# stefanch/sGDML

Measured on AMD Instinct MI355X. Metric: kernel-matrix build+solve wall-clock, N_train=1000 21-atom (aspirin-sized), lower is better.
Workload: dtype f64

## Files before the change

sgdml_amd/csrc/chol.hip:

```cpp
#include "common.h"
#include "tile_sched.h"
#include <array>
#include <type_traits>
#include <utility>

typedef double d4 __attribute__((ext_vector_type(4)));
typedef double d2 __attribute__((ext_vector_type(2)));

#define GT 128
#define GBK 16
#define GPITCH 17

struct GemmArgs {
  const double* A;
  const double* B;
  double* C;
  int64_t M, N, K, lda, ldb, ldc;
  int lower;
  int tiles_m, tiles_n;
  int64_t n_super;
  int64_t s_begin;
  int super_n;
  int aligned;
  int cyc_W, cyc_rank;
  int64_t cyc_lb0, cyc_nb, cyc_col0, cyc_block_rows;
  double* diagA;
  int diag_nbw;
  int64_t diag_off;
  int* diag_info;
  int col0_first;
  int* ready;
  int ready_target, ready_rows;
  const double* A2;
  const double* B2;
  double* C2;
  int64_t M2, N2, K2;
  int tiles2;
  int second_compact;
  int bal;
  TileLaunch tl;
};

__global__ void __launch_bounds__(256, 2) gemm_nt_sub_diag_kernel(GemmArgs g);

template <bool FULL>
__device__ __forceinline__ void gemm_load_tile(const double* __restrict__ G, int64_t ld,
                                               int64_t row0, int64_t nrows, int64_t k0, int64_t K,
                                               int tid, d2 (&r)[4]) {
#pragma unroll
  for (int s = 0; s < 4; ++s) {
    int cidx = tid + 256 * s;
    int row = cidx >> 3, kc = (cidx & 7) * 2;
    int64_t gr = row0 + row, gk = k0 + kc;
    if (FULL) {
      r[s] = *reinterpret_cast<const d2*>(G + gr * ld + gk);
// ... 205 lines not shown
  int64_t ti, tj;
  if (g.bal) {
    if (!tile_decode_bal(g.tl, b, &ti, &tj)) return;
  } else if (!tile_decode_super(b, g.lower, g.col0_first, g.tiles_m, g.tiles_n, g.super_n, g.s_begin, g.n_super, &ti, &tj)) {
    return;
  }
  const int64_t row0 = ti * GT, col0 = tj * GT;
  if (g.cyc_W > 0 && row0 + GT <= g.cyc_block_rows) {
    const int64_t gb = (g.cyc_lb0 + row0 / g.cyc_nb) * g.cyc_W + g.cyc_rank;
    const int64_t grow_last = gb * g.cyc_nb + (row0 + GT - 1) % g.cyc_nb;
    if (g.cyc_col0 + col0 > grow_last) return;
  }
  const bool full = (row0 + GT <= g.M) && (col0 + GT <= g.N) && ((g.K & (GBK - 1)) == 0) && g.aligned;
  if (full)
    gemm_tile_body<true, OW>(g, lds, row0, col0);
  else
    gemm_tile_body<false, OW>(g, lds, row0, col0);
  if (g.ready && g.tiles2 == 0 && ti < g.ready_rows && tj < g.ready_rows) {
    __threadfence();
    __syncthreads();
    if (threadIdx.x == 0) atomicAdd(g.ready, 1);
  }
}

__global__ void __launch_bounds__(256, 2) gemm_nt_sub_kernel(GemmArgs g) {
  __shared__ __attribute__((aligned(16))) double lds[2][2][GT * GPITCH];
  gemm_block<false>(g, lds, blockIdx.x);
}


__global__ void __launch_bounds__(256, 2) gemm_nt_neg_kernel(GemmArgs g) {
  __shared__ __attribute__((aligned(16))) double lds[2][2][GT * GPITCH];
  gemm_block<true>(g, lds, blockIdx.x);
}

struct DiagJob {
  double* A = nullptr;
  int nbw = 0;
  int64_t off = 0;
  int* ready = nullptr;
  int ready_target = 0;
  bool col0_first = false;
  const double* A2 = nullptr;
  const double* B2 = nullptr;
  double* C2 = nullptr;
  int64_t M2 = 0, N2 = 0, K2 = 0;
  int64_t next_M2 = 0, next_N2 = 0, next_K2 = 0;
};

struct TileSchedEntry {
  TileSched S;
  const uint32_t* dev[2] = {nullptr, nullptr};
};
struct TileSchedCache {
  std::map<std::array<int64_t, 7>, TileSchedEntry> entries;
  char* block = nullptr;
  size_t cap = 0, used = 0;
};

void tile_sched_cache_free(gdml_ctx* ctx) {
  if (!ctx->tile_sched) return;
  if (ctx->tile_sched->block) hipFree(ctx->tile_sched->block);
  delete ctx->tile_sched;
  ctx->tile_sched = nullptr;
}

static int second_blocks(int64_t M2, int64_t N2, bool* compact) {
  const int64_t tm2 = ceil_div(M2, GT), tn2 = ceil_div(N2, GT);
  *compact = tm2 >= tn2;
  return (int)(tm2 * tn2 - (*compact ? tn2 * (tn2 - 1) / 2 : 0));
}

static int tile_sched_get(gdml_ctx* ctx, hipStream_t st, int tiles_m, int tiles_n, bool col0_first, int n_launch, int lead2,
                          int64_t K2, int64_t K, const TileSchedEntry** out) {
  *out = nullptr;
  if (!ctx->tile_sched) ctx->tile_sched = new TileSchedCache();
  TileSchedCache* c = ctx->tile_sched;
  const std::array<int64_t, 7> key = {tiles_m, tiles_n, col0_first ? 1 : 0, n_launch, lead2, lead2 ? K2 : 0, lead2 ? K : 0};
  auto it = c->entries.find(key);
  if (it == c->entries.end()) {
    TileSchedEntry e;
    double base[8] = {0, 0, 0, 0, 0, 0, 0, 0};
    for (int q = 0; q < lead2; ++q) base[((q - lead2) % 8 + 8) % 8] += (double)K2 / (double)K;
    tile_sched_build(tiles_m, tiles_n, col0_first, n_launch, base, &e.S);
    if (e.S.ok) {
      const size_t b0 = (e.S.table[0].size() * 4 + 255) & ~(size_t)255, b1 = (e.S.table[1].size() * 4 + 255) & ~(size_t)255;
      const size_t block_bytes = (size_t)8 << 20;
      if (!c->block) {
        HIP_CHECK(ctx, hipMalloc((void**)&c->block, block_bytes));
        c->cap = block_bytes;
      }
      if (b0 + b1 > c->cap) {
        e.S.ok = false;
      } else {
        if (c->used + b0 + b1 > c->cap) {
          HIP_CHECK(ctx, hipDeviceSynchronize());
          c->entries.clear();
          c->used = 0;
        }
        char* d = c->block + c->used;
        c->used += b0 + b1;
        if (!e.S.table[0].empty()) HIP_CHECK(ctx, hipMemcpyAsync(d, e.S.table[0].data(), e.S.table[0].size() * 4, hipMemcpyHostToDevice, st));
        if (!e.S.table[1].empty()) HIP_CHECK(ctx, hipMemcpyAsync(d + b0, e.S.table[1].data(), e.S.table[1].size() * 4, hipMemcpyHostToDevice, st));
        HIP_CHECK(ctx, hipStreamSynchronize(st));
        e.dev[0] = reinterpret_cast<const uint32_t*>(d);
        e.dev[1] = reinterpret_cast<const uint32_t*>(d + b0);
      }
    }
// ... 305 lines not shown
      d4 a[2][4], bb[2][4];
#pragma unroll
      for (int i = 0; i < 2; ++i)
#pragma unroll
        for (int ch = 0; ch < 4; ++ch) {
          a[i][ch] = *reinterpret_cast<const d4*>(Ap + (int64_t)(16 * i) * ld + 16 * ch);
          bb[i][ch] = *reinterpret_cast<const d4*>(Bp + (int64_t)(16 * i) * ld + 16 * ch);
        }
#pragma unroll
      for (int ch = 0; ch < 4; ++ch)
#pragma unroll
        for (int sidx = 0; sidx < 4; ++sidx)
#pragma unroll
          for (int i = 0; i < 2; ++i)
#pragma unroll
            for (int j = 0; j < 2; ++j)
              acc[i][j] = __builtin_amdgcn_mfma_f64_16x16x4f64(-a[i][ch][sidx], bb[j][ch][sidx], acc[i][j], 0, 0, 0);
#pragma unroll
      for (int i = 0; i < 2; ++i)
#pragma unroll
        for (int j = 0; j < 2; ++j)
#pragma unroll
          for (int r = 0; r < 4; ++r) Cp[(int64_t)(16 * i + 4 * r) * ld + 16 * j] = acc[i][j][r];
    }
    __syncthreads();
  }
}


__global__ void __launch_bounds__(256, 2) gemm_nt_sub_diag_kernel(GemmArgs g) {
  __shared__ __attribute__((aligned(16))) double lds[2][2][GT * GPITCH];
  static_assert(sizeof(double) * 2 * 2 * GT * GPITCH >= sizeof(double) * (2 * 64 * 65 + 64 + 128), "LDS of the diagonal role");
  if (blockIdx.x == 0) {
    if (g.ready) {
      if (threadIdx.x == 0) {
        int spins = 0;
        while (__hip_atomic_load(g.ready, __ATOMIC_RELAXED, __HIP_MEMORY_SCOPE_AGENT) < g.ready_target) {
          __builtin_amdgcn_s_sleep(8);
          if (++spins > (1 << 24)) {
            atomicExch(g.ready + 1, 1);
            break;
          }
        }
      }
      __syncthreads();
      __threadfence();
    }
    diag_block_role(g.diagA, g.ldc, g.diag_nbw, g.diag_off, g.diag_info, &lds[0][0][0]);
    return;
  }
  gemm_block<false>(g, lds, (int64_t)blockIdx.x - 1);
}

__global__ void __launch_bounds__(64) potrf64_kernel(double* __restrict__ A, int64_t ld, int w,
                                                     int64_t global_off, int* __restrict__ info) {
  __shared__ __attribute__((aligned(16))) double T[64 * 65];
  __shared__ __attribute__((aligned(16))) double col[64 * 8];
  const int lane = threadIdx.x;
  {
    double tv[64];
    const int lc = lane < w ? lane : w - 1;
#pragma unroll
    for (int r = 0; r < 64; ++r) tv[r] = A[(int64_t)(r < w ? r : w - 1) * ld + lc];
#pragma unroll
    for (int r = 0; r < 64; ++r) T[r * 65 + lane] = (r < w && lane < w) ? tv[r] : ((r == lane) ? 1.0 : 0.0);
  }
  __builtin_amdgcn_s_waitcnt(0xc07f);
  const int fail = potrf64_wave(T, col, lane);
  if (fail != 0 && fail <= w && lane == 0) atomicCAS(info, 0, (int)(global_off + fail));
  for (int r = 0; r < w; ++r)
    if (lane <= r && lane < w) A[(int64_t)r * ld + lane] = T[r * 65 + lane];
}

__global__ void __launch_bounds__(256) potrf_trsm64_kernel(double* __restrict__ A, double* __restrict__ X,
                                                           int64_t ld, int w, int64_t m, int64_t global_off,
                                                           int* __restrict__ info, double* __restrict__ Lsave,
                                                           const double* __restrict__ Lprev,
                                                           double* __restrict__ Aprev, int wprev) {
  __shared__ __attribute__((aligned(16))) double T[64 * 65];
  __shared__ __attribute__((aligned(16))) double Ls[64 * 64];
  __shared__ __attribute__((aligned(16))) double col[64 * 8];
  __shared__ double rinv[64];
  const int tid = threadIdx.x, lane = tid & 63, wave = tid >> 6;
  double pv[16];
  const bool wb = blockIdx.x == 0 && Lprev != nullptr;
  if (wb) {
#pragma unroll
    for (int i = 0; i < 16; ++i) pv[i] = Lprev[tid + 256 * i];
  }
  {
    double tv[16];
    const int lc = lane < w ? lane : w - 1;
#pragma unroll
    for (int i = 0; i < 16; ++i) {
      const int r = wave + 4 * i;
      tv[i] = A[(int64_t)(r < w ? r : w - 1) * ld + lc];
    }
#pragma unroll
    for (int i = 0; i < 16; ++i) {
      const int r = wave + 4 * i;
      T[r * 65 + lane] = (r < w && lane < w) ? tv[i] : ((r == lane) ? 1.0 : 0.0);
    }
  }
  if (wb) {
#pragma unroll
    for (int i = 0; i < 16; ++i) {
// ... 310 lines not shown
                                                            int skip_upper) {
  const int lane = threadIdx.x & 63, wave = threadIdx.x >> 6;
  const int li = lane & 15, lk = lane >> 4;
  const int tn = (ncols + 31) >> 5;
  const int t = blockIdx.x * 4 + wave;
  const int ti = t / tn, tj = t - ti * tn;
  if (32 * ti >= m) return;
  if (skip_upper && tj > ti) return;
  const int r0 = 32 * ti, q0 = 32 * tj;
  d4 acc[2][2], a[2][4], bb[2][4];
  int crow[2][4], ccol[2];
#pragma unroll
  for (int j = 0; j < 2; ++j) ccol[j] = q0 + 16 * j + li;
#pragma unroll
  for (int i = 0; i < 2; ++i)
#pragma unroll
    for (int r = 0; r < 4; ++r) crow[i][r] = r0 + 16 * i + lk + 4 * r;
#pragma unroll
  for (int i = 0; i < 2; ++i) {
    const int ra = r0 + 16 * i + li, rb = q0 + 16 * i + li;
    const double* Ap = A + (int64_t)(ra < m ? ra : m - 1) * ld + 4 * lk;
    const double* Bp = B + (int64_t)(rb < ncols ? rb : ncols - 1) * ld + 4 * lk;
#pragma unroll
    for (int ch = 0; ch < 4; ++ch) {
      a[i][ch] = *reinterpret_cast<const d4*>(Ap + 16 * ch);
      bb[i][ch] = *reinterpret_cast<const d4*>(Bp + 16 * ch);
    }
  }
#pragma unroll
  for (int i = 0; i < 2; ++i)
#pragma unroll
    for (int j = 0; j < 2; ++j)
#pragma unroll
      for (int r = 0; r < 4; ++r) {
        const int rr = crow[i][r] < m ? crow[i][r] : m - 1, cc = ccol[j] < ncols ? ccol[j] : ncols - 1;
        acc[i][j][r] = C[(int64_t)rr * ld + cc];
      }
#pragma unroll
  for (int ch = 0; ch < 4; ++ch)
#pragma unroll
    for (int sidx = 0; sidx < 4; ++sidx)
#pragma unroll
      for (int i = 0; i < 2; ++i)
#pragma unroll
        for (int j = 0; j < 2; ++j)
          acc[i][j] = __builtin_amdgcn_mfma_f64_16x16x4f64(-a[i][ch][sidx], bb[j][ch][sidx], acc[i][j], 0, 0, 0);
#pragma unroll
  for (int i = 0; i < 2; ++i)
#pragma unroll
    for (int j = 0; j < 2; ++j)
#pragma unroll
      for (int r = 0; r < 4; ++r)
        if (crow[i][r] < m && ccol[j] < ncols) C[(int64_t)crow[i][r] * ld + ccol[j]] = acc[i][j][r];
}

int panel_factor_steps(gdml_ctx* ctx, hipStream_t st, double* A, int64_t n, int64_t ld, int64_t k0, int64_t nb);

static int panel_factor(gdml_ctx* ctx, hipStream_t st, double* A, int64_t n, int64_t ld, int64_t k0,
                        int64_t nb) {
  const int64_t below = n - k0 - nb;
  const bool aligned = (reinterpret_cast<uintptr_t>(A) & 31) == 0 && (ld % 4 == 0) && (k0 % 4 == 0);
  if (nb % 64 == 0 && nb <= 512 && below > 0 && aligned) {
    GDML_TRY(panel_factor_steps(ctx, st, A, k0 + nb, ld, k0, nb));
    return launch_panel_trsm(ctx, st, A + k0 * ld + k0, A + (k0 + nb) * ld + k0, ld, (int)nb, below);
  }
  return panel_factor_steps(ctx, st, A, n, ld, k0, nb);
}

int panel_factor_steps(gdml_ctx* ctx, hipStream_t st, double* A, int64_t n, int64_t ld, int64_t k0,
                       int64_t nb) {
  double* save = nullptr;
  GDML_TRY(ctx_slot(ctx, SLOT_PANEL_SAVE, 2 * 4096 * 8, &save));
  const double* Lprev = nullptr;
  double* Aprev = nullptr;
  int wprev = 0, flip = 0;
  for (int64_t jj = 0; jj < nb; jj += 64) {
    const int64_t c0 = k0 + jj;
    const int w = (int)((nb - jj < 64) ? nb - jj : 64);
    double* Ad = A + c0 * ld + c0;
    const int64_t m = n - c0 - w;
    if (m > 0) {
      double* X = A + (c0 + w) * ld + c0;
      double* Lsave = save + flip * 4096;
      hipLaunchKernelGGL(potrf_trsm64_kernel, dim3((unsigned)ceil_div(m, 256)), dim3(256), 0, st, Ad, X, ld, w, m,
                         c0, ctx->d_info, Lsave, Lprev, Aprev, wprev);
      ctx->launch_counter++;
      Lprev = Lsave;
      Aprev = Ad;
      wprev = w;
      flip ^= 1;
      const int64_t ncols = k0 + nb - (c0 + w);
      if (ncols > 0) {
        const bool al32 = (reinterpret_cast<uintptr_t>(X) & 31) == 0 && (ld % 4 == 0);
        if (w == 64 && m <= 2048 && al32) {
          const int tiles = (int)(ceil_div(m, 32) * ceil_div(ncols, 32));
          hipLaunchKernelGGL(rank64_update_kernel, dim3((unsigned)ceil_div(tiles, 4)), dim3(256), 0, st, X, X,
                             A + (c0 + w) * ld + (c0 + w), ld, (int)m, (int)ncols, 1);
          ctx->launch_counter++;
        } else {
          GDML_TRY(launch_gemm_nt_sub(ctx, st, X, ld, X, ld, A + (c0 + w) * ld + (c0 + w), ld, m, ncols, w, 0));
        }
      }
    } else {
      if (Lprev) {
        hipLaunchKernelGGL(writeback_block_kernel, dim3(1), dim3(256), 0, st, Lprev, Aprev, ld, wprev);
        ctx->launch_counter++;
        Lprev = nullptr;
      }
      hipLaunchKernelGGL(potrf64_kernel, dim3(1), dim3(64), 0, st, Ad, ld, w, c0, ctx->d_info);
      ctx->launch_counter++;
    }
  }
  if (Lprev) {
    hipLaunchKernelGGL(writeback_block_kernel, dim3(1), dim3(256), 0, st, Lprev, Aprev, ld, wprev);
    ctx->launch_counter++;
  }
  return GDML_OK;
}

int chol_factor_device(gdml_ctx* ctx, double* A, int64_t n, int64_t ld, int* info_out, int64_t n_rows) {
  if (n_rows < n) n_rows = n;
  HIP_CHECK(ctx, hipMemsetAsync(ctx->d_info, 0, sizeof(int), ctx->stream));
  int64_t NB = (int64_t)ctx_opt(ctx, "chol.nb", 512);
  if (NB < 64 || NB % 64 || NB > 512) NB = 512;
  hipStream_t st = ctx->stream;
  int64_t min_rows = (int64_t)ctx_opt(ctx, "chol.fused_min_rows", 12288);
  if (min_rows < 1) min_rows = 1;
  int64_t OB = (int64_t)ctx_opt(ctx, "chol.outer", 1024);
  if (OB != 2 * NB || NB % GT != 0) OB = NB;
  const int64_t outer_min_rows = (int64_t)ctx_opt(ctx, "chol.outer_min_rows", 16384);
  auto width_at = [&](int64_t c0) -> int64_t {
    const int64_t left = n - (c0 + OB);
    const int64_t w = (OB > NB && left > 0 && left >= outer_min_rows) ? OB : NB;
    return (n - c0 < w) ? n - c0 : w;
  };
  int64_t k0 = 0, nb = (n < NB) ? n : NB;
  int ready_count = 0;
  HIP_CHECK(ctx, hipMemsetAsync(ctx->d_info + 6, 0, 2 * sizeof(int), ctx->stream));
  GDML_TRY(panel_factor(ctx, st, A, n_rows, ld, 0, nb));
  for (;;) {
    const int64_t t0 = k0 + nb;
    if (t0 >= n) break;
    const int64_t nb2 = width_at(t0);
    const int64_t t1 = t0 + nb2;
    const double* P = A + t0 * ld + k0;
    const bool fuse = (nb2 % 64 == 0) && (n - t1 >= min_rows) && (n_rows - t1 > 0);
    if (fuse && nb2 == 2 * NB) {
      const int64_t ta = t0 + NB;
      const int64_t sm = (ceil_div(n_rows - t0, GT) + 7) / 8, n_super_all = sm * (sm + 1) / 2;
      int64_t s_split = n_super_all / 2;
      if (s_split < sm) s_split = sm;
      const double fs = ((double)s_split + 0.5) / (double)n_super_all;
      DiagJob dj;
      dj.A = A + t0 * ld + t0; dj.nbw = (int)(NB / 64); dj.off = t0;
      dj.col0_first = true;
      dj.ready = ctx->d_info + 6;
      const int block_tiles = (int)((NB / GT) * (NB / GT + 1) / 2);
      ready_count += block_tiles;
      dj.ready_target = ready_count;
      dj.next_M2 = n_rows - ta; dj.next_N2 = NB; dj.next_K2 = NB;
      GDML_TRY(launch_gemm_nt_sub_part(ctx, st, P, ld, P, ld, A + t0 * ld + t0, ld, n_rows - t0, n - t0, nb, 1, 0.0, fs, true,
                                       &dj));
      double* Xa = A + ta * ld + t0;
      GDML_TRY(launch_panel_trsm(ctx, st, A + t0 * ld + t0, Xa, ld, (int)NB, n_rows - ta));
      dj.A = A + ta * ld + ta; dj.off = ta;
      dj.A2 = Xa; dj.B2 = Xa; dj.C2 = A + ta * ld + ta; dj.M2 = n_rows - ta; dj.N2 = NB; dj.K2 = NB;
      ready_count += block_tiles;
      dj.ready_target = ready_count;
      GDML_TRY(launch_gemm_nt_sub_part(ctx, st, P, ld, P, ld, A + t0 * ld + t0, ld, n_rows - t0, n - t0, nb, 1, fs, 1.0, true,
                                       &dj));
      GDML_TRY(launch_panel_trsm(ctx, st, A + ta * ld + ta, A + t1 * ld + ta, ld, (int)NB, n_rows - t1));
    } else {
      GDML_TRY(launch_gemm_nt_sub(ctx, st, P, ld, P, ld, A + t0 * ld + t0, ld, n_rows - t0, nb2, nb, 0));
      const double* P1 = A + t1 * ld + k0;
      if (fuse) {
        DiagJob dj;
        dj.A = A + t0 * ld + t0;
        dj.nbw = (int)(nb2 / 64);
        dj.off = t0;
        GDML_TRY(launch_gemm_nt_sub_part(ctx, st, P1, ld, P1, ld, A + t1 * ld + t1, ld, n_rows - t1, n - t1, nb, 1, 0.0,
                                         1.0, true, &dj));
        GDML_TRY(launch_panel_trsm(ctx, st, A + t0 * ld + t0, A + t1 * ld + t0, ld, (int)nb2, n_rows - t1));
      } else if (t1 < n) {
        hipStream_t sp = ctx->stream2;
        HIP_CHECK(ctx, hipEventRecord(ctx->ev_la[0], st));
        HIP_CHECK(ctx, hipStreamWaitEvent(sp, ctx->ev_la[0], 0));
        GDML_TRY(panel_factor(ctx, sp, A, n_rows, ld, t0, nb2));
        HIP_CHECK(ctx, hipEventRecord(ctx->ev_la[1], sp));
        GDML_TRY(launch_gemm_nt_sub(ctx, st, P1, ld, P1, ld, A + t1 * ld + t1, ld, n_rows - t1, n - t1, nb, 1));
        HIP_CHECK(ctx, hipStreamWaitEvent(st, ctx->ev_la[1], 0));
      } else {
        GDML_TRY(panel_factor(ctx, st, A, n_rows, ld, t0, nb2));
      }
    }
    k0 = t0;
    nb = nb2;
  }
  HIP_CHECK(ctx, hipGetLastError());
  int info8[8] = {0};
  HIP_CHECK(ctx, hipMemcpyAsync(info8, ctx->d_info, sizeof(info8), hipMemcpyDeviceToHost, ctx->stream));
  HIP_CHECK(ctx, hipStreamSynchronize(ctx->stream));
  if (info8[7] != 0)
    return gdml_fail(ctx, GDML_ERR_HIP, "Cholesky: the diagonal-block workgroup gave up waiting for its tiles (schedule bug)");
  if (info_out) *info_out = info8[0];
  return GDML_OK;
}

template <bool TRANS>
__device__ __forceinline__ double tri_solve64_wave(const double* Ls, double b, int lane) {
  double v[64];
#pragma unroll
  for (int k = 0; k < 64; ++k) v[k] = TRANS ? Ls[k * 65 + lane] : Ls[lane * 65 + k];
  double sol = 0.0;
  if (!TRANS) {
#pragma unroll
    for (int c = 0; c < 64; ++c) {
      const double t = b / v[c];
      const double zc = __shfl(t, c, 64);
      if (lane == c) sol = zc;
      b -= v[c] * zc;
    }
  } else {
#pragma unroll
    for (int r = 63; r >= 0; --r) {
      const double t = b / v[r];
      const double xr = __shfl(t, r, 64);
      if (lane == r) sol = xr;
      b -= v[r] * xr;
    }
  }
  return sol;
}

__device__ __forceinline__ void load_block64(const double* __restrict__ L, int64_t ld, int64_t c0,
                                             int w, double* Ls, int tid, int T) {
  for (int e = tid; e < 64 * 64; e += T) {
    int r = e >> 6, c = e & 63;
    double v = (r == c) ? 1.0 : 0.0;
    if (r < w && c < w && c <= r) v = L[(c0 + r) * ld + c0 + c];
    Ls[r * 65 + c] = v;
  }
}

__global__ void __launch_bounds__(256) trsv_fwd_kernel(const double* __restrict__ L, int64_t ld,
                                                       int64_t n, int64_t c0, int w,
                                                       double* __restrict__ b,
                                                       double* __restrict__ z_out) {
  __shared__ __attribute__((aligned(16))) double Ls[64 * 65];
  __shared__ double z[64];
// ... 284 lines not shown
```

sgdml_amd/csrc/ctx.hip:

```cpp
#include <stdarg.h>

#include <mutex>

#include "common.h"

static std::string g_create_err;

int gdml_fail(gdml_ctx* ctx, int code, const char* fmt, ...) {
  char buf[1024];
  va_list ap;
  va_start(ap, fmt);
  vsnprintf(buf, sizeof(buf), fmt, ap);
  va_end(ap);
  if (ctx)
    ctx->err = buf;
  else
    g_create_err = buf;
  return code;
}

extern "C" int gdml_abi_version(void) { return 4; }

static const char* kKnownOptions[] = {
    "asm.wave", "asm.j_chunk", "asm.lower", "asm.strip", "asm.i_chunk",
    "asm.pts", "asm.pts_nv", "asm.pts_nt", "asm.pts_xcd", "asm.pts_i_chunk", "asm.pts_debug", "asm.perm_debug", "asm.perm_w", "asm.perm_lds_kb", "asm.perm_level", "asm.perm_nimg", "asm.perm_pg", "asm.perm_na", "asm.perm_fast_store", "asm.perm_i_chunk", "asm.perm_compact", "asm.perm_lds_rows", "asm.big1", "asm.perm2", "asm.perm2_min_n", "asm.perm2_min_p", "asm.perm2_split", "asm.perm2_post", "asm.perm2_ed", "asm.perm2_es", "asm.perm2_direct", "asm.perm2_chunk", "asm.perm2_i_chunk", "asm.perm2_debug",
    "nys.trsm_left", "nys.syrk_split", "predict.wide_pad", "predict.tn_fill", "chol.nb", "pcg.gemv_plain",
    "chol.fused_min_rows", "chol.outer", "chol.outer_min_rows", "gemm.balance", "trsm.debug",
    "trsv.persist", "predict.wave_only", "predict.mfma", "predict.fill", "predict.mfma_wide", "predict.fused", "predict.fused_rows", "predict.fused_spin",
    "lu.nb", "comm.force_collectives", "nys.force_qr", "nys.force_fail", "dist.nb", "dist.lookahead", "dist.force_panels", "pcg.depth", "pcg.precon_form", "pcg.f32_rows_per", "pcg.f32_rw", "pcg.f32_min_pivot", "pcg.f32_last_min_pivot", "pcg.f32_gram_rows", "pcg.f32_inplace",
    "predict.hess_generic", "predict.hess_chunk_rows", "predict.cov_chunk", "predict.cov_global", "predict.cov_few_rows", "predict.cov_few_split_timers", "predict.md_chunk_frames", "predict.md_fused", "predict.pimd_tile", "predict.relax_fused", "predict.relax_chunk_steps", "predict.vib_chunk", "chol.loo_chunk", "chol.extend_chunk", "chol.remove_chunk", "chol.select_chunk", "chol.select_mem_budget",
    "chol.evidence_chunk", "chol.evidence_mem_budget", "chol.evidence_global"};

double ctx_opt(const gdml_ctx* ctx, const char* key, double dflt) {
  auto it = ctx->opts.find(key);
  return it == ctx->opts.end() ? dflt : it->second;
}

extern "C" int gdml_set_option(gdml_ctx* ctx, const char* key, double value) {
  if (!ctx || !key) return GDML_ERR_INVALID;
  for (const char* k : kKnownOptions)
    if (strcmp(k, key) == 0) {
      ctx->opts[key] = value;
      return GDML_OK;
    }
  return gdml_fail(ctx, GDML_ERR_INVALID, "gdml_set_option: unknown option '%s'", key);
}

extern "C" int gdml_get_option(gdml_ctx* ctx, const char* key, double* value_out, int* is_set_out) {
  if (!ctx || !key) return GDML_ERR_INVALID;
  auto it = ctx->opts.find(key);
  if (value_out) *value_out = it == ctx->opts.end() ? 0.0 : it->second;
  if (is_set_out) *is_set_out = it != ctx->opts.end();
  return GDML_OK;
}

static void options_from_env(gdml_ctx* ctx) {
  const char* e = getenv("GDML_OPTIONS");
  if (!e) return;
  std::string s(e);
  size_t pos = 0;
  while (pos < s.size()) {
    size_t end = s.find(',', pos);
    if (end == std::string::npos) end = s.size();
    const std::string kv = s.substr(pos, end - pos);
    const size_t eq = kv.find('=');
    if (eq != std::string::npos) (void)gdml_set_option(ctx, kv.substr(0, eq).c_str(), atof(kv.c_str() + eq + 1));
    pos = end + 1;
  }
}

struct ArenaBlock {
  int64_t off, bytes;
  gdml_ctx* owner;
};
struct DeviceArena {
  void* base = nullptr;
  int64_t bytes = 0;
  std::vector<ArenaBlock> blocks;
};
static DeviceArena g_arena[64];
// ... 432 lines not shown
```

sgdml_amd/csrc/tile_sched.h:

```cpp
#pragma once
#include <math.h>
#include <stdint.h>
#include <vector>

#if defined(__HIPCC__)
#define TS_HD __host__ __device__ __forceinline__
#else
#define TS_HD inline
#endif

TS_HD void ts_tri(int64_t t, int64_t* I, int64_t* J) {
  int64_t i = (int64_t)((sqrt(8.0 * (double)t + 1.0) - 1.0) * 0.5);
  while (i * (i + 1) / 2 > t) --i;
  while ((i + 1) * (i + 2) / 2 <= t) ++i;
  *I = i;
  *J = t - i * (i + 1) / 2;
}

TS_HD bool tile_decode_super(int64_t b, int lower, int col0_first, int tiles_m, int tiles_n, int super_n, int64_t s_begin,
                             int64_t n_super, int64_t* ti_out, int64_t* tj_out) {
  const int64_t xcd = b & 7, loc = b >> 3;
  const int64_t s = s_begin + (loc >> 6) * 8 + xcd;
  const int within = (int)(loc & 63);
  if (s >= n_super) return false;
// ... 180 lines not shown
    L.r1 = (l == last) ? (int)R : (int)r_cut;
    L.nh = nh;
    L.col0_first = col0_first ? 1 : 0;
    int64_t per[8], mx = 0, cnt_max = 0;
    for (int x = 0; x < 8; ++x) {
      const int64_t h = (l == 0) ? (int64_t)dh.t[x].size() : 0, t = (l == last) ? (int64_t)dt.t[x].size() : 0;
      if (h > 0xffff || t > 0xffff) return;
      L.hn[x >> 2] |= (uint64_t)h << (16 * (x & 3));
      L.tn[x >> 2] |= (uint64_t)t << (16 * (x & 3));
      per[x] = h + t;
      if (per[x] > mx) mx = per[x];
      const int64_t c = per[x] + (int64_t)(L.r1 - L.r0) * 64;
      if (c > cnt_max) cnt_max = c;
    }
    L.stride = (int)mx;
    S->table[l].assign((size_t)(8 * mx), 0);
    for (int x = 0; x < 8; ++x) {
      size_t o = (size_t)x * (size_t)mx;
      if (l == 0) for (uint32_t v : dh.t[x]) S->table[l][o++] = v;
      if (l == last) for (uint32_t v : dt.t[x]) S->table[l][o++] = v;
    }
    S->blocks[l] = 8 * cnt_max;
    auto count = [&](int64_t ti, int64_t tj) {
      const bool lastrow = ti == tiles_m - 1;
      ++S->tiles[l];
      if (ti == tj) ++(lastrow ? S->diag_last[l] : S->diag_int[l]);
      else ++(lastrow ? S->off_last[l] : S->off_int[l]);
    };
    for (int x = 0; x < 8; ++x) {
      if (l == 0) for (uint32_t v : dh.t[x]) count(v & 0xffff, v >> 16);
      if (l == last) for (uint32_t v : dt.t[x]) count(v & 0xffff, v >> 16);
    }
    for (int64_t ff = (int64_t)L.r0 * 8; ff < (int64_t)L.r1 * 8; ++ff) {
      int64_t SI, SJ;
      ts_full_super(ff, L.col0_first, L.nh, &SI, &SJ);
      for (int r = 0; r < 8; ++r)
        for (int c = 0; c < 8; ++c) count(SI * 8 + r, SJ * 8 + c);
    }
  }
  S->ok = true;
}

inline double tile_sched_counted_flops(const TileSched& S, int l, int64_t M, int64_t K, int tiles_m, int gt) {
  const double rl = (double)(M - (int64_t)(tiles_m - 1) * gt), g = (double)gt;
  return (double)K * (2.0 * g * g * (double)S.off_int[l] + 2.0 * rl * g * (double)S.off_last[l] +
                      g * (g + 1.0) * (double)S.diag_int[l] + rl * (rl + 1.0) * (double)S.diag_last[l]);
}
inline double tile_sched_flops(const TileSched& S, int l, int64_t M, int64_t K, int tiles_m, int gt) {
  if (l < S.n_launch - 1) return tile_sched_counted_flops(S, l, M, K, tiles_m, gt);
  double before = 0.0;
  for (int i = 0; i < l; ++i) before += tile_sched_counted_flops(S, i, M, K, tiles_m, gt);
  return (double)M * (double)(M + 1) * (double)K - before;
}
```

Before: 1.264.

## Add planned deep-lookahead Cholesky with segmented multi-GEMM launches balanced across XCDs

Replaces the inline blocked-Cholesky loop with a precomputed, cached op plan. In a deep window (chol.deep columns), trailing updates from several outer panels are deferred into a pooled far-field GEMM. Those tiles are then spread across the paired per-step launches through a new segmented kernel. That kernel reads per-XCD tile tables, runs up to three GEMM segments in one launch and keeps the spin-waiting diagonal-factor block. The aim is to cut repeated full trailing-update sweeps, launch count and load imbalance across the eight XCDs, at the cost of complex scheduling, a one-off host plan build with device upload, and more deferred-work bookkeeping.

Result: faster. 1.247 (median of 6 runs) (-1.4%).

```diff
diff --git a/sgdml_amd/csrc/chol.hip b/sgdml_amd/csrc/chol.hip
--- a/sgdml_amd/csrc/chol.hip
+++ b/sgdml_amd/csrc/chol.hip
@@ -1,6 +1,7 @@
 #include "common.h"
 #include "tile_sched.h"
 #include <array>
+#include <memory>
 #include <type_traits>
 #include <utility>
 
@@ -312,8 +313,10 @@
   TileSched S;
   const uint32_t* dev[2] = {nullptr, nullptr};
 };
+struct CholPlanEntry;
 struct TileSchedCache {
   std::map<std::array<int64_t, 7>, TileSchedEntry> entries;
+  std::vector<std::pair<std::array<int64_t, 8>, std::shared_ptr<CholPlanEntry>>> plans;
   char* block = nullptr;
   size_t cap = 0, used = 0;
 };
@@ -725,6 +728,66 @@
   gemm_block<false>(g, lds, (int64_t)blockIdx.x - 1);
 }
 
+struct SegArgs {
+  const double* A[3];
+  const double* B[3];
+  double* C[3];
+  int64_t M[3], N[3], K[3];
+  int64_t ld;
+  const uint32_t* table;
+  int stride;
+  uint64_t cnt[4];
+  double* diagA;
+  int diag_nbw;
+  int64_t diag_off;
+  int* diag_info;
+  int* ready;
+  int ready_target;
+};
+
+__global__ void __launch_bounds__(256, 2) gemm_nt_sub_seg_kernel(SegArgs s) {
+  __shared__ __attribute__((aligned(16))) double lds[2][2][GT * GPITCH];
+  if (blockIdx.x == 0) {
+    if (threadIdx.x == 0) {
+      int spins = 0;
+      while (__hip_atomic_load(s.ready, __ATOMIC_RELAXED, __HIP_MEMORY_SCOPE_AGENT) < s.ready_target) {
+        __builtin_amdgcn_s_sleep(8);
+        if (++spins > (1 << 24)) {
+          atomicExch(s.ready + 1, 1);
+          break;
+        }
+      }
+    }
+    __syncthreads();
+    __threadfence();
+    diag_block_role(s.diagA, s.ld, s.diag_nbw, s.diag_off, s.diag_info, &lds[0][0][0]);
+    return;
+  }
+  const int64_t b = (int64_t)blockIdx.x - 1;
+  const int x = (int)(b & 7);
+  const int64_t pos = b >> 3;
+  if (pos >= (int64_t)((s.cnt[x >> 1] >> (32 * (x & 1))) & 0xffffffffu)) return;
+  const uint32_t v = __builtin_amdgcn_readfirstlane(s.table[(int64_t)x * s.stride + pos]);
+  const int si = TS_SEG_ID(v);
+  GemmArgs h;
+  h.A = s.A[0]; h.B = s.B[0]; h.C = s.C[0]; h.M = s.M[0]; h.N = s.N[0]; h.K = s.K[0];
+  if (si == 1) { h.A = s.A[1]; h.B = s.B[1]; h.C = s.C[1]; h.M = s.M[1]; h.N = s.N[1]; h.K = s.K[1]; }
+  if (si == 2) { h.A = s.A[2]; h.B = s.B[2]; h.C = s.C[2]; h.M = s.M[2]; h.N = s.N[2]; h.K = s.K[2]; }
+  h.lda = h.ldb = h.ldc = s.ld;
+  const int64_t row0 = TS_SEG_TI(v) * GT, col0 = TS_SEG_TJ(v) * GT;
+  const bool aligned = ((reinterpret_cast<uintptr_t>(h.A) | reinterpret_cast<uintptr_t>(h.B)) & 15) == 0 && (s.ld % 2 == 0);
+  const bool full = (row0 + GT <= h.M) && (col0 + GT <= h.N) && ((h.K & (GBK - 1)) == 0) && aligned;
+  if (full)
+    gemm_tile_body<true, false>(h, lds, row0, col0);
+  else
+    gemm_tile_body<false, false>(h, lds, row0, col0);
+  if (TS_SEG_COUNTED(v)) {
+    __threadfence();
+    __syncthreads();
+    if (threadIdx.x == 0) atomicAdd(s.ready, 1);
+  }
+}
+
 __global__ void __launch_bounds__(64) potrf64_kernel(double* __restrict__ A, int64_t ld, int w,
                                                      int64_t global_off, int* __restrict__ info) {
   __shared__ __attribute__((aligned(16))) double T[64 * 65];
@@ -1141,6 +1204,90 @@
 #pragma unroll
       for (int r = 0; r < 4; ++r)
         if (crow[i][r] < m && ccol[j] < ncols) C[(int64_t)crow[i][r] * ld + ccol[j]] = acc[i][j][r];
+}
+
+struct CholPlanEntry {
+  CholPlan plan;
+  uint32_t* block = nullptr;
+  std::vector<const uint32_t*> dev;
+  std::vector<int> stride;
+  ~CholPlanEntry() {
+    if (block) (void)hipFree(block);
+  }
+};
+
+static int chol_plan_get(gdml_ctx* ctx, hipStream_t st, int64_t n, int64_t n_rows, CholPlanOpts po, std::shared_ptr<CholPlanEntry>* out) {
+  if (!ctx->tile_sched) ctx->tile_sched = new TileSchedCache();
+  TileSchedCache* c = ctx->tile_sched;
+  const std::array<int64_t, 8> key = {n, n_rows, po.NB, po.OB, po.outer_min_rows, po.fused_min_rows, po.deep, po.deep_min_rows};
+  for (auto& kv : c->plans)
+    if (kv.first == key) { *out = kv.second; return GDML_OK; }
+  auto e = std::make_shared<CholPlanEntry>();
+  chol_plan_build(n, n_rows, po, &e->plan);
+  *out = e;
+  if (e->plan.segs.empty()) return GDML_OK;
+  std::vector<uint32_t> host;
+  std::vector<size_t> at;
+  for (const PlanSegLaunch& L : e->plan.segs) {
+    const size_t stride = plan_launch_stride(L);
+    at.push_back(host.size());
+    e->stride.push_back((int)stride);
+    host.resize(host.size() + plan_launch_words(L), 0);
+    for (int x = 0; x < 8; ++x) std::copy(L.xcd[x].begin(), L.xcd[x].end(), host.begin() + at.back() + x * stride);
+  }
+  if (hipMalloc((void**)&e->block, host.size() * 4) != hipSuccess) {
+    (void)hipGetLastError();
+    e->block = nullptr;
+    po.deep = 0;
+    e->plan = CholPlan();
+    e->stride.clear();
+    chol_plan_build(n, n_rows, po, &e->plan);
+    return GDML_OK;
+  }
+  HIP_CHECK(ctx, hipMemcpyAsync(e->block, host.data(), host.size() * 4, hipMemcpyHostToDevice, st));
+  HIP_CHECK(ctx, hipStreamSynchronize(st));
+  for (size_t o : at) e->dev.push_back(e->block + o);
+  if (c->plans.size() >= 4) c->plans.erase(c->plans.begin());
+  c->plans.emplace_back(key, e);
+  return GDML_OK;
+}
+
+static int launch_gemm_seg(gdml_ctx* ctx, hipStream_t st, double* A, int64_t ld, const CholPlanEntry& pe, int idx, int ready_target) {
+  const PlanSegLaunch& L = pe.plan.segs[idx];
+  SegArgs s = {};
+  for (int i = 0; i < 3; ++i) {
+    const PlanSeg& g = L.seg[i];
+    s.A[i] = A + g.origin * ld + g.a_col0;
+    s.B[i] = s.A[i];
+    s.C[i] = A + g.origin * ld + g.origin;
+    s.M[i] = g.M; s.N[i] = g.N; s.K[i] = g.K;
+  }
+  s.ld = ld;
+  s.table = pe.dev[idx];
+  s.stride = pe.stride[idx];
+  int64_t mx = 0;
+  for (int x = 0; x < 8; ++x) {
+    const int64_t cnt = (int64_t)L.xcd[x].size();
+    s.cnt[x >> 1] |= (uint64_t)cnt << (32 * (x & 1));
+    if (cnt > mx) mx = cnt;
+  }
+  s.diagA = A + L.diag0 * ld + L.diag0;
+  s.diag_nbw = L.diag_nbw;
+  s.diag_off = L.diag0;
+  s.diag_info = ctx->d_info;
+  s.ready = ctx->d_info + 6;
+  s.ready_target = ready_target;
+  const int slot = (st == (ctx->kt_stream ? ctx->kt_stream : ctx->stream)) ? ktime_begin(ctx) : -1;
+  hipLaunchKernelGGL(gemm_nt_sub_seg_kernel, dim3((unsigned)(8 * mx + 1)), dim3(256), 0, st, s);
+  ktime_end(ctx, slot, "gemm_nt_sub_diag", L.flops);
+  if (slot >= 0 && L.far_tiles > 0) {
+    KernelStat& k = ctx->kstats["gemm_nt_sub_deep"];
+    k.launches += 1;
+    k.work += L.far_flops;
+  }
+  ctx->launch_counter++;
+  HIP_CHECK(ctx, hipGetLastError());
+  return GDML_OK;
 }
 
 int panel_factor_steps(gdml_ctx* ctx, hipStream_t st, double* A, int64_t n, int64_t ld, int64_t k0, int64_t nb);
@@ -1215,62 +1362,71 @@
   hipStream_t st = ctx->stream;
   int64_t min_rows = (int64_t)ctx_opt(ctx, "chol.fused_min_rows", 12288);
   if (min_rows < 1) min_rows = 1;
-  int64_t OB = (int64_t)ctx_opt(ctx, "chol.outer", 1024);
-  if (OB != 2 * NB || NB % GT != 0) OB = NB;
   const int64_t outer_min_rows = (int64_t)ctx_opt(ctx, "chol.outer_min_rows", 16384);
-  auto width_at = [&](int64_t c0) -> int64_t {
-    const int64_t left = n - (c0 + OB);
-    const int64_t w = (OB > NB && left > 0 && left >= outer_min_rows) ? OB : NB;
-    return (n - c0 < w) ? n - c0 : w;
-  };
-  int64_t k0 = 0, nb = (n < NB) ? n : NB;
+  CholPlanOpts po;
+  po.NB = NB; po.OB = (int64_t)ctx_opt(ctx, "chol.outer", 1024); po.outer_min_rows = outer_min_rows; po.fused_min_rows = min_rows;
+  po.deep = (int64_t)ctx_opt(ctx, "chol.deep", 4096);
+  po.deep_min_rows = (int64_t)ctx_opt(ctx, "chol.deep_min_rows", 26624);
+  std::shared_ptr<CholPlanEntry> pe;
+  GDML_TRY(chol_plan_get(ctx, st, n, n_rows, po, &pe));
   int ready_count = 0;
   HIP_CHECK(ctx, hipMemsetAsync(ctx->d_info + 6, 0, 2 * sizeof(int), ctx->stream));
-  GDML_TRY(panel_factor(ctx, st, A, n_rows, ld, 0, nb));
-  for (;;) {
-    const int64_t t0 = k0 + nb;
-    if (t0 >= n) break;
-    const int64_t nb2 = width_at(t0);
-    const int64_t t1 = t0 + nb2;
+  const int block_tiles = (int)((NB / GT) * (NB / GT + 1) / 2);
+  for (const CholOp& c : pe->plan.ops) {
+    const int64_t k0 = c.k0, nb = c.nb, t0 = c.t0, nb2 = c.nb2, t1 = t0 + nb2;
     const double* P = A + t0 * ld + k0;
-    const bool fuse = (nb2 % 64 == 0) && (n - t1 >= min_rows) && (n_rows - t1 > 0);
-    if (fuse && nb2 == 2 * NB) {
-      const int64_t ta = t0 + NB;
-      const int64_t sm = (ceil_div(n_rows - t0, GT) + 7) / 8, n_super_all = sm * (sm + 1) / 2;
-      int64_t s_split = n_super_all / 2;
-      if (s_split < sm) s_split = sm;
-      const double fs = ((double)s_split + 0.5) / (double)n_super_all;
-      DiagJob dj;
-      dj.A = A + t0 * ld + t0; dj.nbw = (int)(NB / 64); dj.off = t0;
-      dj.col0_first = true;
-      dj.ready = ctx->d_info + 6;
-      const int block_tiles = (int)((NB / GT) * (NB / GT + 1) / 2);
-      ready_count += block_tiles;
-      dj.ready_target = ready_count;
-      dj.next_M2 = n_rows - ta; dj.next_N2 = NB; dj.next_K2 = NB;
-      GDML_TRY(launch_gemm_nt_sub_part(ctx, st, P, ld, P, ld, A + t0 * ld + t0, ld, n_rows - t0, n - t0, nb, 1, 0.0, fs, true,
-                                       &dj));
-      double* Xa = A + ta * ld + t0;
-      GDML_TRY(launch_panel_trsm(ctx, st, A + t0 * ld + t0, Xa, ld, (int)NB, n_rows - ta));
-      dj.A = A + ta * ld + ta; dj.off = ta;
-      dj.A2 = Xa; dj.B2 = Xa; dj.C2 = A + ta * ld + ta; dj.M2 = n_rows - ta; dj.N2 = NB; dj.K2 = NB;
-      ready_count += block_tiles;
-      dj.ready_target = ready_count;
-      GDML_TRY(launch_gemm_nt_sub_part(ctx, st, P, ld, P, ld, A + t0 * ld + t0, ld, n_rows - t0, n - t0, nb, 1, fs, 1.0, true,
-                                       &dj));
-      GDML_TRY(launch_panel_trsm(ctx, st, A + ta * ld + ta, A + t1 * ld + ta, ld, (int)NB, n_rows - t1));
-    } else {
-      GDML_TRY(launch_gemm_nt_sub(ctx, st, P, ld, P, ld, A + t0 * ld + t0, ld, n_rows - t0, nb2, nb, 0));
-      const double* P1 = A + t1 * ld + k0;
-      if (fuse) {
+    const double* P1 = A + t1 * ld + k0;
+    switch (c.kind) {
+      case OP_PANEL:
+        GDML_TRY(panel_factor(ctx, st, A, n_rows, ld, t0, nb2));
+        break;
+      case OP_TRSM:
+        GDML_TRY(launch_panel_trsm(ctx, st, A + t0 * ld + t0, A + t1 * ld + t0, ld, (int)nb2, n_rows - t1));
+        break;
+      case OP_PAIR1:
+      case OP_PAIR2: {
+        const int64_t ta = t0 + NB;
+        const int64_t sm = (ceil_div(n_rows - t0, GT) + 7) / 8, n_super_all = sm * (sm + 1) / 2;
+        int64_t s_split = n_super_all / 2;
+        if (s_split < sm) s_split = sm;
+        const double fs = ((double)s_split + 0.5) / (double)n_super_all;
+        DiagJob dj;
+        dj.nbw = (int)(NB / 64);
+        dj.col0_first = true;
+        dj.ready = ctx->d_info + 6;
+        ready_count += block_tiles;
+        dj.ready_target = ready_count;
+        dj.next_M2 = n_rows - ta; dj.next_N2 = NB; dj.next_K2 = NB;
+        if (c.kind == OP_PAIR1) {
+          dj.A = A + t0 * ld + t0; dj.off = t0;
+          GDML_TRY(launch_gemm_nt_sub_part(ctx, st, P, ld, P, ld, A + t0 * ld + t0, ld, n_rows - t0, n - t0, nb, 1, 0.0, fs, true,
+                                           &dj));
+        } else {
+          double* Xa = A + ta * ld + t0;
+          dj.A = A + ta * ld + ta; dj.off = ta;
+          dj.A2 = Xa; dj.B2 = Xa; dj.C2 = A + ta * ld + ta; dj.M2 = n_rows - ta; dj.N2 = NB; dj.K2 = NB;
+          GDML_TRY(launch_gemm_nt_sub_part(ctx, st, P, ld, P, ld, A + t0 * ld + t0, ld, n_rows - t0, n - t0, nb, 1, fs, 1.0, true,
+                                           &dj));
+        }
+        break;
+      }
+      case OP_SEG:
+        ready_count += block_tiles;
+        GDML_TRY(launch_gemm_seg(ctx, st, A, ld, *pe, c.seg, ready_count));
+        break;
+      case OP_RECT:
+        GDML_TRY(launch_gemm_nt_sub(ctx, st, P, ld, P, ld, A + t0 * ld + t0, ld, n_rows - t0, nb2, nb, 0));
+        break;
+      case OP_FUSED: {
         DiagJob dj;
         dj.A = A + t0 * ld + t0;
         dj.nbw = (int)(nb2 / 64);
         dj.off = t0;
         GDML_TRY(launch_gemm_nt_sub_part(ctx, st, P1, ld, P1, ld, A + t1 * ld + t1, ld, n_rows - t1, n - t1, nb, 1, 0.0,
                                          1.0, true, &dj));
-        GDML_TRY(launch_panel_trsm(ctx, st, A + t0 * ld + t0, A + t1 * ld + t0, ld, (int)nb2, n_rows - t1));
-      } else if (t1 < n) {
+        break;
+      }
+      case OP_TAIL: {
         hipStream_t sp = ctx->stream2;
         HIP_CHECK(ctx, hipEventRecord(ctx->ev_la[0], st));
         HIP_CHECK(ctx, hipStreamWaitEvent(sp, ctx->ev_la[0], 0));
@@ -1278,12 +1434,9 @@
         HIP_CHECK(ctx, hipEventRecord(ctx->ev_la[1], sp));
         GDML_TRY(launch_gemm_nt_sub(ctx, st, P1, ld, P1, ld, A + t1 * ld + t1, ld, n_rows - t1, n - t1, nb, 1));
         HIP_CHECK(ctx, hipStreamWaitEvent(st, ctx->ev_la[1], 0));
-      } else {
-        GDML_TRY(panel_factor(ctx, st, A, n_rows, ld, t0, nb2));
-      }
-    }
-    k0 = t0;
-    nb = nb2;
+        break;
+      }
+    }
   }
   HIP_CHECK(ctx, hipGetLastError());
   int info8[8] = {0};
diff --git a/sgdml_amd/csrc/ctx.hip b/sgdml_amd/csrc/ctx.hip
--- a/sgdml_amd/csrc/ctx.hip
+++ b/sgdml_amd/csrc/ctx.hip
@@ -25,7 +25,7 @@
     "asm.wave", "asm.j_chunk", "asm.lower", "asm.strip", "asm.i_chunk",
     "asm.pts", "asm.pts_nv", "asm.pts_nt", "asm.pts_xcd", "asm.pts_i_chunk", "asm.pts_debug", "asm.perm_debug", "asm.perm_w", "asm.perm_lds_kb", "asm.perm_level", "asm.perm_nimg", "asm.perm_pg", "asm.perm_na", "asm.perm_fast_store", "asm.perm_i_chunk", "asm.perm_compact", "asm.perm_lds_rows", "asm.big1", "asm.perm2", "asm.perm2_min_n", "asm.perm2_min_p", "asm.perm2_split", "asm.perm2_post", "asm.perm2_ed", "asm.perm2_es", "asm.perm2_direct", "asm.perm2_chunk", "asm.perm2_i_chunk", "asm.perm2_debug",
     "nys.trsm_left", "nys.syrk_split", "predict.wide_pad", "predict.tn_fill", "chol.nb", "pcg.gemv_plain",
-    "chol.fused_min_rows", "chol.outer", "chol.outer_min_rows", "gemm.balance", "trsm.debug",
+    "chol.fused_min_rows", "chol.outer", "chol.outer_min_rows", "chol.deep", "chol.deep_min_rows", "gemm.balance", "trsm.debug",
     "trsv.persist", "predict.wave_only", "predict.mfma", "predict.fill", "predict.mfma_wide", "predict.fused", "predict.fused_rows", "predict.fused_spin",
     "lu.nb", "comm.force_collectives", "nys.force_qr", "nys.force_fail", "dist.nb", "dist.lookahead", "dist.force_panels", "pcg.depth", "pcg.precon_form", "pcg.f32_rows_per", "pcg.f32_rw", "pcg.f32_min_pivot", "pcg.f32_last_min_pivot", "pcg.f32_gram_rows", "pcg.f32_inplace",
     "predict.hess_generic", "predict.hess_chunk_rows", "predict.cov_chunk", "predict.cov_global", "predict.cov_few_rows", "predict.cov_few_split_timers", "predict.md_chunk_frames", "predict.md_fused", "predict.pimd_tile", "predict.relax_fused", "predict.relax_chunk_steps", "predict.vib_chunk", "chol.loo_chunk", "chol.extend_chunk", "chol.remove_chunk", "chol.select_chunk", "chol.select_mem_budget",
diff --git a/sgdml_amd/csrc/tile_sched.h b/sgdml_amd/csrc/tile_sched.h
--- a/sgdml_amd/csrc/tile_sched.h
+++ b/sgdml_amd/csrc/tile_sched.h
@@ -256,3 +256,321 @@
   for (int i = 0; i < l; ++i) before += tile_sched_counted_flops(S, i, M, K, tiles_m, gt);
   return (double)M * (double)(M + 1) * (double)K - before;
 }
+
+#define TS_SEG_TI(v) ((int64_t)((v) & 0x3fffu))
+#define TS_SEG_TJ(v) ((int64_t)(((v) >> 14) & 0x3fffu))
+#define TS_SEG_ID(v) ((int)(((v) >> 28) & 7u))
+#define TS_SEG_COUNTED(v) ((v) >> 31)
+
+struct CholPlanOpts {
+  int64_t NB = 512, OB = 1024, outer_min_rows = 16384, fused_min_rows = 12288, deep = 0, deep_min_rows = 26624;
+};
+struct PlanSeg {
+  int64_t origin = 0, a_col0 = 0, M = 0, N = 0, K = 0;
+  int kind = 0;
+};
+struct PlanSegLaunch {
+  PlanSeg seg[3];
+  std::vector<uint32_t> xcd[8];
+  int64_t diag0 = 0;
+  int diag_nbw = 0, counted = 0;
+  int64_t tiles = 0, far_tiles = 0;
+  double flops = 0.0, far_flops = 0.0, cost = 0.0;
+};
+enum { OP_PANEL = 0, OP_RECT, OP_PAIR1, OP_PAIR2, OP_FUSED, OP_TRSM, OP_TAIL, OP_SEG };
+struct CholOp {
+  int kind = 0;
+  int64_t k0 = 0, nb = 0;
+  int64_t t0 = 0, nb2 = 0;
+  int seg = -1;
+};
+struct CholPlan {
+  std::vector<CholOp> ops;
+  std::vector<PlanSegLaunch> segs;
+  int64_t NB = 0, OB = 0, deep = 0, deep_end = 0;
+};
+
+namespace cp_detail {
+const int GT_ = 128;
+const int64_t TURNOVER = 66;
+struct Unit {
+  uint32_t v = 0;
+  int64_t K = 0;
+  uint8_t seg = 0, kind = 0;
+  bool full = false, ragged = false, first = false;
+  int tiles() const { return full ? 64 : 1; }
+  int64_t cost() const { return (int64_t)tiles() * (K + TURNOVER); }
+  uint32_t tile(int i) const { return full ? v + (uint32_t)(i >> 3) + ((uint32_t)(i & 7) << 14) : v; }
+};
+template <class Pred>
+inline void gen_units(int seg, const PlanSeg& s, Pred pred, bool first, std::vector<Unit>* out, int tj_lo = 0, int tj_hi = 1 << 30,
+                      bool last_row = false) {
+  const int tiles_m = (int)((s.M + GT_ - 1) / GT_), tiles_n = (int)((s.N + GT_ - 1) / GT_);
+  const bool ragged = (s.M % GT_) != 0 || (s.N % GT_) != 0;
+  const int sm = (tiles_m + 7) / 8;
+  Unit u;
+  u.seg = (uint8_t)seg; u.kind = (uint8_t)s.kind; u.K = s.K; u.first = first;
+  const int sj_lo = tj_lo / 8, sj_hi = tj_hi > (1 << 29) ? (1 << 29) : (tj_hi + 7) / 8;
+  for (int SI = 0; SI < sm; ++SI)
+    for (int SJ = 0; SJ <= SI; ++SJ) {
+      if ((SJ < sj_lo || SJ >= sj_hi) && !(last_row && SI == sm - 1)) continue;
+      uint32_t got[64];
+      int ng = 0;
+      for (int r = 0; r < 8; ++r)
+        for (int c = 0; c < 8; ++c) {
+          const int ti = SI * 8 + r, tj = SJ * 8 + c;
+          if (ti < tiles_m && tj < tiles_n && tj <= ti && pred(ti, tj)) got[ng++] = (uint32_t)ti | ((uint32_t)tj << 14);
+        }
+      if (ng == 64 && !(ragged && SI * 8 + 7 == tiles_m - 1)) {
+        u.full = true; u.ragged = false; u.v = got[0];
+        out->push_back(u);
+        continue;
+      }
+      for (int i = 0; i < ng; ++i) {
+        u.full = false; u.v = got[i];
+        u.ragged = ragged && (int)TS_SEG_TI(got[i]) == tiles_m - 1;
+        out->push_back(u);
+      }
+    }
+}
+inline int64_t units_cost(const std::vector<Unit>& v, size_t from = 0) {
+  int64_t c = 0;
+  for (size_t i = from; i < v.size(); ++i) c += v[i].cost();
+  return c;
+}
+inline void deal_launch(const std::vector<Unit>& units, int counted_seg, int counted_rows, PlanSegLaunch* L) {
+  std::vector<Unit> cls[5];
+  for (const Unit& u : units) cls[u.first ? 0 : (u.kind == 1 ? 1 : (u.ragged ? 2 : (u.full ? 3 : 4)))].push_back(u);
+  int64_t load[8] = {0, 0, 0, 0, 0, 0, 0, 0};
+  auto put = [&](int x, const Unit& u) {
+    const PlanSeg& s = L->seg[u.seg];
+    for (int i = 0; i < u.tiles(); ++i) {
+      const uint32_t v = u.tile(i);
+      const int64_t ti = TS_SEG_TI(v), tj = TS_SEG_TJ(v);
+      const bool cnt = u.seg == counted_seg && ti < counted_rows && tj < counted_rows;
+      L->xcd[x].push_back(v | ((uint32_t)u.seg << 28) | (cnt ? 0x80000000u : 0u));
+      const double r = (double)(s.M - ti * GT_ < GT_ ? s.M - ti * GT_ : GT_), c = (double)(s.N - tj * GT_ < GT_ ? s.N - tj * GT_ : GT_);
+      const double fl = (double)s.K * ((ti == tj && s.kind != 2) ? r * (r + 1.0) : 2.0 * r * c);
+      L->flops += fl; ++L->tiles;
+      if (s.kind == 1) { L->far_flops += fl; ++L->far_tiles; }
+    }
+    load[x] += u.cost();
+  };
+  std::vector<Unit> fulls, singles;
+  for (int c = 0; c < 5; ++c) {
+    fulls.clear(); singles.clear();
+    size_t n_full = 0, nf = 0;
+    for (const Unit& u : cls[c]) n_full += u.full ? 1 : 0;
+    const size_t keep = n_full - n_full % 8;
+    for (const Unit& u : cls[c]) {
+      if (u.full && nf++ < keep) { fulls.push_back(u); continue; }
+      Unit w = u;
+      w.full = false;
+      for (int i = 0; i < u.tiles(); ++i) { w.v = u.tile(i); singles.push_back(w); }
+    }
+    auto deal_full = [&]() {
+      for (const Unit& u : fulls) {
+        int best = 0;
+        for (int x = 1; x < 8; ++x) if (load[x] < load[best]) best = x;
+        put(best, u);
+      }
+    };
+    if (c != 0) deal_full();
+    int64_t tot = 0;
+    for (const Unit& u : singles) tot += u.cost();
+    for (int x = 0; x < 8; ++x) tot += load[x];
+    const double mean = (double)tot / 8.0;
+    size_t i = 0;
+    for (int x = 0; x < 8; ++x) {
+      double want = mean - (double)load[x];
+      while (i < singles.size() && (x == 7 || want >= 0.5 * (double)singles[i].cost())) {
+        want -= (double)singles[i].cost();
+        put(x, singles[i++]);
+      }
+    }
+    if (c == 0) deal_full();
+  }
+  int64_t mx = 0;
+  for (int x = 0; x < 8; ++x) if (load[x] > mx) mx = load[x];
+  L->cost = (double)mx;
+}
+}
+
+inline size_t plan_launch_stride(const PlanSegLaunch& L) {
+  size_t mx = 0;
+  for (int x = 0; x < 8; ++x) mx = L.xcd[x].size() > mx ? L.xcd[x].size() : mx;
+  return mx;
+}
+inline size_t plan_launch_words(const PlanSegLaunch& L) { return (8 * plan_launch_stride(L) + 63) & ~(size_t)63; }
+
+inline void chol_plan_build(int64_t n, int64_t n_rows, CholPlanOpts o, CholPlan* P) {
+  using namespace cp_detail;
+  *P = CholPlan();
+  if (n_rows < n) n_rows = n;
+  int64_t NB = o.NB;
+  if (NB < 64 || NB % 64 || NB > 512) NB = 512;
+  int64_t min_rows = o.fused_min_rows < 1 ? 1 : o.fused_min_rows;
+  int64_t OB = o.OB;
+  if (OB != 2 * NB || NB % GT_ != 0) OB = NB;
+  P->NB = NB; P->OB = OB;
+  auto width_at = [&](int64_t c0) -> int64_t {
+    const int64_t left = n - (c0 + OB);
+    const int64_t w = (OB > NB && left > 0 && left >= o.outer_min_rows) ? OB : NB;
+    return (n - c0 < w) ? n - c0 : w;
+  };
+  auto fuse_at = [&](int64_t t0) {
+    const int64_t nb2 = width_at(t0), t1 = t0 + nb2;
+    return (nb2 % 64 == 0) && (n - t1 >= min_rows) && (n_rows - t1 > 0);
+  };
+  auto paired = [&](int64_t t0) { return t0 < n && OB == 2 * NB && width_at(t0) == 2 * NB && fuse_at(t0); };
+  int64_t W = (OB == 2 * NB) ? o.deep : 0;
+  if (W > 0) W -= W % OB;
+  int64_t X = NB;
+  if (W >= OB && n_rows / GT_ < 0x3ff0) {
+    while (paired(X) && paired(X + OB) && n - X >= o.deep_min_rows) X += OB;
+  }
+  const bool has_deep = X > NB;
+  P->deep = has_deep ? W : 0;
+  P->deep_end = has_deep ? X : 0;
+  const int OBt = (int)(OB / GT_), NBt = (int)(NB / GT_);
+  const int block_tiles = NBt * (NBt + 1) / 2;
+  auto op = [&](int kind, int64_t k0, int64_t nb, int64_t t0, int64_t nb2, int seg = -1) {
+    CholOp c;
+    c.kind = kind; c.k0 = k0; c.nb = nb; c.t0 = t0; c.nb2 = nb2; c.seg = seg;
+    P->ops.push_back(c);
+  };
+  int64_t S = 0, E = NB + W;
+  PlanSeg pool_seg;
+  std::vector<Unit> pool;
+  size_t pool_at = 0;
+  int64_t span_cost = 0;
+  int span_left = 0;
+  auto near_seg = [&](int64_t t0, int64_t k0, int64_t nb) {
+    PlanSeg s;
+    s.origin = t0; s.a_col0 = k0; s.M = n_rows - t0; s.N = n - t0; s.K = nb; s.kind = 0;
+    return s;
+  };
+  auto second_seg = [&](int64_t t0) {
+    PlanSeg s;
+    s.origin = t0 + NB; s.a_col0 = t0; s.M = n_rows - (t0 + NB); s.N = NB; s.K = NB; s.kind = 2;
+    return s;
+  };
+  auto near_bound = [&](int64_t t0, int64_t blockS, int64_t blockE) -> int { return (t0 == blockS && blockS > 0) ? 0 : (int)((blockE - t0) / GT_); };
+  auto near_pred = [&](const PlanSeg& s, int bound) {
+    const int tiles_m = (int)((s.M + GT_ - 1) / GT_);
+    const bool ragged = (s.M % GT_) != 0 || (s.N % GT_) != 0;
+    return [=](int ti, int tj) { return tj < bound || (ragged && ti == tiles_m - 1); };
+  };
+  auto far_pred = [&](const PlanSeg& s) {
+    const int tiles_m = (int)((s.M + GT_ - 1) / GT_);
+    const bool ragged = (s.M % GT_) != 0 || (s.N % GT_) != 0;
+    return [=](int ti, int tj) { return !(ragged && ti == tiles_m - 1); };
+  };
+  auto step_fixed_cost = [&](int64_t t0, int64_t nb, int64_t blockS, int64_t blockE) {
+    std::vector<Unit> u;
+    const PlanSeg s = near_seg(t0, t0 - nb, nb), s2 = second_seg(t0);
+    const int bound = near_bound(t0, blockS, blockE);
+    gen_units(0, s, near_pred(s, bound), false, &u, 0, bound, true);
+    gen_units(2, s2, [](int, int) { return true; }, true, &u, 0, NBt);
+    return units_cost(u);
+  };
+
+  int64_t k0 = 0, nb = (n < NB) ? n : NB;
+  op(OP_PANEL, 0, 0, 0, nb);
+  for (;;) {
+    const int64_t t0 = k0 + nb;
+    if (t0 >= n) break;
+    const int64_t nb2 = width_at(t0), t1 = t0 + nb2;
+    const bool fuse = fuse_at(t0);
+    if (fuse && nb2 == 2 * NB && has_deep && t0 <= X) {
+      const int64_t ta = t0 + NB;
+      int must = 0;
+      if (t0 == E) {
+        pool_seg = PlanSeg();
+        pool_seg.origin = E; pool_seg.a_col0 = S; pool_seg.M = n_rows - E; pool_seg.N = n - E; pool_seg.K = E - S; pool_seg.kind = 1;
+        S = E; E = S + W;
+        int m = 0;
+        int64_t fixed = 0;
+        for (int64_t t = t0; t < E && (t < X || t == t0); t += OB) { ++m; fixed += step_fixed_cost(t, t == t0 ? nb : OB, S, E); }
+        must = (m > 1) ? (int)(W / GT_) : OBt;
+        pool.clear(); pool_at = 0;
+        const auto fp = far_pred(pool_seg);
+        gen_units(1, pool_seg, [&](int ti, int tj) { return fp(ti, tj) && tj < OBt; }, true, &pool, 0, OBt);
+        gen_units(1, pool_seg, [&](int ti, int tj) { return fp(ti, tj) && tj >= OBt && tj < must; }, false, &pool, OBt, must);
+        gen_units(1, pool_seg, [&](int ti, int tj) { return fp(ti, tj) && tj >= must; }, false, &pool, must);
+        span_cost = fixed + units_cost(pool);
+        span_left = 2 * m;
+      } else if (t0 == X) {
+        pool.clear(); pool_at = 0;
+        pool_seg = PlanSeg();
+        if (E < n) {
+          pool_seg.origin = E; pool_seg.a_col0 = S; pool_seg.M = n_rows - E; pool_seg.N = n - E; pool_seg.K = X - S; pool_seg.kind = 1;
+          gen_units(1, pool_seg, far_pred(pool_seg), false, &pool);
+        }
+        span_cost = step_fixed_cost(t0, nb, S, E) + units_cost(pool);
+        span_left = 2;
+      } else if (span_left == 0) {
+        span_cost = step_fixed_cost(t0, nb, S, E);
+        span_left = 2;
+      }
+      const PlanSeg ns = near_seg(t0, k0, nb);
+      const int bound = near_bound(t0, S, E);
+      const auto np_ = near_pred(ns, bound);
+      std::vector<Unit> rest;
+      size_t rest_at = 0;
+      for (int l = 0; l < 2; ++l) {
+        PlanSegLaunch L;
+        L.seg[0] = ns;
+        L.seg[1] = pool_seg;
+        if (l == 1) L.seg[2] = second_seg(t0);
+        std::vector<Unit> u;
+        if (l == 0) {
+          gen_units(0, ns, [&](int ti, int tj) { return np_(ti, tj) && tj < OBt; }, true, &u, 0, OBt);
+          while (pool_at < pool.size() && must > 0 && (int)TS_SEG_TJ(pool[pool_at].v) < must) u.push_back(pool[pool_at++]);
+          rest.clear(); rest_at = 0;
+          gen_units(0, ns, [&](int ti, int tj) { return np_(ti, tj) && tj >= OBt; }, false, &rest, OBt, bound, true);
+        } else {
+          gen_units(2, L.seg[2], [](int, int) { return true; }, true, &u, 0, NBt);
+        }
+        int64_t cost = units_cost(u);
+        const int64_t target = span_cost / span_left;
+        if (l == 0) {
+          while (rest_at < rest.size() && cost + rest[rest_at].cost() / 2 <= target) { cost += rest[rest_at].cost(); u.push_back(rest[rest_at++]); }
+        } else {
+          while (rest_at < rest.size()) { cost += rest[rest_at].cost(); u.push_back(rest[rest_at++]); }
+        }
+        while (pool_at < pool.size() && (span_left == 1 || cost + pool[pool_at].cost() / 2 <= target)) {
+          cost += pool[pool_at].cost();
+          u.push_back(pool[pool_at++]);
+        }
+        span_cost -= cost;
+        --span_left;
+        L.diag0 = (l == 0) ? t0 : ta;
+        L.diag_nbw = (int)(NB / 64);
+        L.counted = block_tiles;
+        const bool counted_in_pool = (l == 0) && bound == 0;
+        deal_launch(u, l == 1 ? 2 : (counted_in_pool ? 1 : 0), NBt, &L);
+        P->segs.push_back(std::move(L));
+        op(OP_SEG, k0, nb, t0, nb2, (int)P->segs.size() - 1);
+        op(OP_TRSM, 0, 0, l == 0 ? t0 : ta, NB);
+      }
+    } else if (fuse && nb2 == 2 * NB) {
+      op(OP_PAIR1, k0, nb, t0, nb2);
+      op(OP_TRSM, 0, 0, t0, NB);
+      op(OP_PAIR2, k0, nb, t0, nb2);
+      op(OP_TRSM, 0, 0, t0 + NB, NB);
+    } else {
+      op(OP_RECT, k0, nb, t0, nb2);
+      if (fuse) {
+        op(OP_FUSED, k0, nb, t0, nb2);
+        op(OP_TRSM, 0, 0, t0, nb2);
+      } else if (t1 < n) {
+        op(OP_TAIL, k0, nb, t0, nb2);
+      } else {
+        op(OP_PANEL, 0, 0, t0, nb2);
+      }
+    }
+    k0 = t0;
+    nb = nb2;
+  }
+}
```
